# ChikaYan/mvs_gaussian_splatting

Hardware: AMD Instinct MI355X
Metric: Mpixels/s fwd + train-step ms @1080p, 6M Gaussians, 1->8 MI355X (higher is better)
Workload: dtype f32

## Files before the change

### include/gsr.h

```cpp
#ifndef GSR_H_
#define GSR_H_

#include <stddef.h>
#include <stdint.h>

#ifdef __cplusplus
extern "C" {
#endif

#define GSR_ABI_VERSION 16

enum {
  GSR_OK = 0,
  GSR_E_BADARG = -1,
  GSR_E_CAPACITY = -2,
  GSR_E_ALIGN = -3
};

typedef struct GsrParams {
  int32_t P;
  int32_t M;
  int32_t D;
  int32_t width, height;
  float tan_fovx, tan_fovy;
  float scale_modifier;
  int32_t prefiltered;
  int32_t debug;
  const float* means3D;
  const float* shs;
  const float* colors_precomp;
  const float* opacities;
  const float* scales;
  const float* rotations;
  const float* cov3D_precomp;
  const float* viewmatrix;
  const float* projmatrix;
  const float* campos;
  const float* bg;
  void* profile;
  const float* shs_rest;
  int32_t act_flags;
  int32_t binning_mode;
  uint32_t* counts_pinned;
  int32_t forward_only;
  int32_t debug_flags;
  uint8_t* visible_out;
  int32_t depth_span_lt24;
} GsrParams;

enum {
  GSR_DEBUG_NO_MINIBLOCK_CULL = 1
};

enum {
  GSR_BINNING_TWO_LEVEL = 0,
  GSR_BINNING_KEYS64 = 1,
  GSR_BINNING_TWO_LEVEL_CULLED = 2
};

enum {
  GSR_ACT_SCALE_EXP = 1,
  GSR_ACT_ROT_NORMALIZE = 2,
  GSR_ACT_OPACITY_SIGMOID = 4
};

typedef struct GsrGrads {
  float* dL_dmeans3D;
  float* dL_dmeans2D;
  float* dL_dshs;
  float* dL_dcolors;
  float* dL_dopacities;
  float* dL_dscales;
  float* dL_drotations;
  float* dL_dcov3D;
  float* dL_dshs_rest;
  float* stats_xyz_gradient_accum;
  float* stats_denom;
  float* stats_max_radii2D;
} GsrGrads;

int gsr_abi_version(void);
const char* gsr_last_error(void);
const char* gsr_build_info(void);

// ... 191 lines not shown
```

### mvs_gaussian_splatting_amd/_lib.py

```python
from __future__ import annotations

import ctypes as C
import os
import threading

_HERE = os.path.dirname(os.path.abspath(__file__))
LIB_PATH = os.environ.get("GSR_LIB_PATH") or os.path.join(_HERE, "libgsr_hip.so")

ABI_VERSION = 16


class GsrParams(C.Structure):
    _fields_ = [
        ("P", C.c_int32), ("M", C.c_int32), ("D", C.c_int32),
        ("width", C.c_int32), ("height", C.c_int32),
        ("tan_fovx", C.c_float), ("tan_fovy", C.c_float), ("scale_modifier", C.c_float),
        ("prefiltered", C.c_int32), ("debug", C.c_int32),
        ("means3D", C.c_void_p), ("shs", C.c_void_p), ("colors_precomp", C.c_void_p),
        ("opacities", C.c_void_p), ("scales", C.c_void_p), ("rotations", C.c_void_p),
        ("cov3D_precomp", C.c_void_p), ("viewmatrix", C.c_void_p), ("projmatrix", C.c_void_p),
        ("campos", C.c_void_p), ("bg", C.c_void_p), ("profile", C.c_void_p),
        ("shs_rest", C.c_void_p), ("act_flags", C.c_int32), ("binning_mode", C.c_int32),
        ("counts_pinned", C.c_void_p), ("forward_only", C.c_int32), ("debug_flags", C.c_int32),
        ("visible_out", C.c_void_p), ("depth_span_lt24", C.c_int32),
    ]


class GsrGrads(C.Structure):
    _fields_ = [
        ("dL_dmeans3D", C.c_void_p), ("dL_dmeans2D", C.c_void_p), ("dL_dshs", C.c_void_p),
        ("dL_dcolors", C.c_void_p), ("dL_dopacities", C.c_void_p), ("dL_dscales", C.c_void_p),
        ("dL_drotations", C.c_void_p), ("dL_dcov3D", C.c_void_p), ("dL_dshs_rest", C.c_void_p),
        ("stats_xyz_gradient_accum", C.c_void_p), ("stats_denom", C.c_void_p), ("stats_max_radii2D", C.c_void_p),
    ]


class GsrGrow(C.Structure):
    _fields_ = [("P", C.c_int32), ("G", C.c_int32), ("mode", C.c_int32), ("num_dirs", C.c_int32), ("n_rest", C.c_int32)] + [
        (n, C.c_void_p) for n in ("xyz", "f_dc", "f_rest", "opacity", "scaling", "rotation", "dirs_prob", "dirs",
                                  "conti_dirs", "grow_dist", "split_distance", "split_scale", "noise", "vidx", "src")]


class GsrGrowGrads(C.Structure):
    _fields_ = [("in_", C.c_void_p * 7), ("out", C.c_void_p * 7)] + [
        (n, C.c_void_p) for n in ("d_dirs_prob", "d_conti_dirs", "d_grow_dist", "d_split_distance", "d_split_scale")]


GROW_DIR, GROW_CONTINUOUS, GROW_DISTANCE, SPLIT_DISTANCE, SPLIT_SCALE = 1, 2, 4, 8, 16


class GsrDensifyFork(C.Structure):
    _fields_ = [("P", C.c_int32), ("mode", C.c_int32), ("num_dirs", C.c_int32)] + [
        (n, C.c_void_p) for n in ("xyz", "scaling", "rotation", "dirs_prob", "dirs", "conti_dirs", "grow_dist",
                                  "split_distance", "split_scale", "noise", "dir_noise")]


DENSIFY_GROW, DENSIFY_SYMMETRIC = 32, 64
ROW_COPY, ROW_CONST, ROW_SKIP = 0, 1, 2


def ROW_POLICY(orig_sel: int, extra: int, child: int) -> int:
    return orig_sel | (extra << 2) | (child << 4)
ACT_SCALE_EXP, ACT_ROT_NORMALIZE, ACT_OPACITY_SIGMOID = 1, 2, 4
BINNING_TWO_LEVEL, BINNING_KEYS64, BINNING_TWO_LEVEL_CULLED = 0, 1, 2
DSSIM_ONE_MINUS_MEAN, DSSIM_CLAMPED_HALF = 0, 1
DEBUG_NO_MINIBLOCK_CULL = 1


ADAM_MAX_TENSORS = 16


class GsrAdamTensor(C.Structure):
    _fields_ = [("param", C.c_void_p), ("grad", C.c_void_p), ("exp_avg", C.c_void_p), ("exp_avg_sq", C.c_void_p),
                ("numel", C.c_int64)] + [
        (n, C.c_float) for n in ("lerp_weight", "beta2", "sq_weight", "bc2_sqrt", "eps", "step_size")]


class GsrAdamBatch(C.Structure):
    _fields_ = [("count", C.c_int32), ("reserved", C.c_int32), ("t", GsrAdamTensor * ADAM_MAX_TENSORS)]


SYMBOLS = {
    "gsr_abi_version": (C.c_int, []),
    "gsr_last_error": (C.c_char_p, []),
    "gsr_build_info": (C.c_char_p, []),
    "gsr_geom_bytes": (C.c_size_t, [C.c_int32]),
    "gsr_image_bytes": (C.c_size_t, [C.c_int32, C.c_int32]),
    "gsr_binning_bytes": (C.c_size_t, [C.c_uint32, C.c_uint32, C.c_int32, C.c_int32, C.c_int32]),
    "gsr_backward_bytes": (C.c_size_t, [C.c_int32, C.c_uint32]),
    "gsr_forward_preprocess": (C.c_int, [C.POINTER(GsrParams), C.c_void_p, C.c_void_p, C.c_void_p,
                                         C.POINTER(C.c_uint32), C.POINTER(C.c_uint32)]),
    "gsr_forward_render": (C.c_int, [C.POINTER(GsrParams), C.c_void_p, C.c_void_p, C.c_size_t, C.c_void_p,
                                     C.c_uint32, C.c_uint32, C.c_void_p, C.c_void_p]),
    "gsr_forward": (C.c_int, [C.POINTER(GsrParams), C.c_void_p, C.c_void_p, C.c_size_t, C.c_uint32, C.c_void_p,
                              C.c_void_p, C.c_void_p, C.c_void_p, C.c_void_p]),
    "gsr_event_create": (C.c_int, [C.POINTER(C.c_void_p)]),
    "gsr_event_destroy": (C.c_int, [C.c_void_p]),
    "gsr_event_wait": (C.c_int, [C.c_void_p]),
    "gsr_event_query": (C.c_int, [C.c_void_p, C.POINTER(C.c_int32)]),
# ... 144 lines not shown
```

### mvs_gaussian_splatting_amd/csrc/gsr_api.hip

```cpp
#include <hip/hip_runtime.h>
#include <dlfcn.h>
#include <stdio.h>
#include <string.h>
#include <atomic>
#include <mutex>
#include <string>
#include <vector>

#include "gsr_common.h"
#include "gsr_launch.h"

using namespace gsr;

namespace {
thread_local std::string g_err = "";

int fail(int code, const char* msg) {
  g_err = msg;
  return code;
}
int hip_fail(hipError_t e, const char* where) {
  g_err = std::string(where) + ": " + hipGetErrorString(e);
  return (int)e;
}
// ... 441 lines not shown
                 uint32_t R, uint32_t V, const float* dL_dout_color, void* bwd_ws, size_t bwd_ws_bytes,
                 const GsrGrads* grads, void* stream) {
  if (p && p->forward_only) return fail(GSR_E_BADARG, "the forward ran with forward_only = 1: no state for a backward");
  if (int rc = validate(p)) return rc;
  if (!grads) return fail(GSR_E_BADARG, "grads is NULL");
  if (p->P == 0) return 0;
  if (!radii || !geom_ws || !img_ws || !dL_dout_color || !bwd_ws) return fail(GSR_E_BADARG, "NULL workspace / input");
  if (!grads->dL_dmeans3D || !grads->dL_dmeans2D || !grads->dL_dopacities)
    return fail(GSR_E_BADARG, "dL_dmeans3D / dL_dmeans2D / dL_dopacities must be non-NULL");
  if (p->shs && !grads->dL_dshs) return fail(GSR_E_BADARG, "dL_dshs required with shs");
  if (p->shs_rest && !grads->dL_dshs_rest) return fail(GSR_E_BADARG, "dL_dshs_rest required with shs_rest");
  if (p->shs_rest && ((uintptr_t)grads->dL_dshs_rest & 15u) != 0) return fail(GSR_E_ALIGN, "dL_dshs_rest must be 16-byte aligned");
  if (p->shs && !p->shs_rest && p->M == 16 && ((uintptr_t)grads->dL_dshs & 15u) != 0)
    return fail(GSR_E_ALIGN, "dL_dshs must be 16-byte aligned");
  if (p->colors_precomp && !grads->dL_dcolors) return fail(GSR_E_BADARG, "dL_dcolors required with colors_precomp");
  {
    const int n_stats = (grads->stats_xyz_gradient_accum != nullptr) + (grads->stats_denom != nullptr) +
                        (grads->stats_max_radii2D != nullptr);
    if (n_stats != 0 && n_stats != 3) return fail(GSR_E_BADARG, "the three stats_* pointers must be given together");
  }
  const BwdLayout Wl(p->P, R);
  if (bwd_ws_bytes < Wl.bytes) return fail(GSR_E_CAPACITY, "backward workspace too small");
  if (((uintptr_t)bwd_ws & 255u) != 0) return fail(GSR_E_ALIGN, "bwd_ws must be 256-byte aligned");
  hipStream_t s = static_cast<hipStream_t>(stream);
  const GeomLayout L(p->P);
  const ImageLayout I(p->width, p->height);
  GradRow* rows = at<GradRow>(bwd_ws, Wl.rows);
  uint8_t* flags = at<uint8_t>(bwd_ws, Wl.flags);
  const GeomRec* rec = at<GeomRec>(geom_ws, L.rec);
  if (R > 0) {
    if (!bin_ws) return fail(GSR_E_BADARG, "bin_ws is NULL");
    const SortedViews sv = sorted_views(bin_ws, R, V, p->width, p->height, p->binning_mode);
    const uint32_t* point_list = sv.point_list;
    GSR_HIP(hipMemsetAsync(flags, 0, R, s));
    {
      StageTimer t(p, GSR_STAGE_RENDER_BWD, s);
      launch_render_bwd(p->width, p->height, at<uint2>(img_ws, I.ranges), point_list, rec,
                        at<uint32_t>(geom_ws, L.slot_base), p->bg,
                        at<float>(img_ws, I.final_T), at<uint32_t>(img_ws, I.n_contrib),
                        at<uint32_t>(img_ws, I.tile_max), dL_dout_color, rows, flags,
                        at<uint32_t>(img_ws, I.tile_order), s, sv.inst_mask);
    }
    if (int rc = check(p, s, "render_bwd")) return rc;
  }
  {
    StageTimer t(p, GSR_STAGE_PREPROCESS_BWD, s);
    launch_sum_big_rows(at<uint32_t>(geom_ws, L.total) + TOTAL_BIG, at<uint32_t>(geom_ws, L.block_big_offs), L.nblocks,
                        at<uint32_t>(geom_ws, L.big_list), rec, at<uint32_t>(geom_ws, L.slot_base), rows, flags, s);
    launch_preprocess_bwd(*p, radii, rec, at<uint32_t>(geom_ws, L.slot_base), rows, flags, *grads, s);
  }
  return check(p, s, "preprocess_bwd");
}

int gsr_profile_create(void** handle) {
  if (!handle) return fail(GSR_E_BADARG, "handle is NULL");
  *handle = new Profile();
  return 0;
}
int gsr_profile_destroy(void* handle) {
  Profile* pr = static_cast<Profile*>(handle);
  if (!pr) return 0;
  for (auto& sp : pr->used) { if (sp.a) (void)hipEventDestroy(sp.a); if (sp.b) (void)hipEventDestroy(sp.b); }
  for (auto e : pr->pool) (void)hipEventDestroy(e);
  delete pr;
  return 0;
}
int gsr_profile_collect(void* handle, double* ms_sum, uint32_t* counts) {
  Profile* pr = static_cast<Profile*>(handle);
  if (!pr || !ms_sum || !counts) return fail(GSR_E_BADARG, "NULL argument");
  std::vector<Profile::Span> spans;
  {
    std::lock_guard<std::mutex> lock(pr->mu);
    spans.swap(pr->used);
  }
// ... 400 lines not shown
```

### mvs_gaussian_splatting_amd/csrc/gsr_common.h

```cpp
#pragma once
#include <hip/hip_runtime.h>
#include <stdint.h>
#include "../../include/gsr.h"

namespace gsr {

constexpr int TILE = 16;
constexpr int WAVE = 64;
constexpr float NEAR_Z = 0.2f;
constexpr float DILATION = 0.3f;
constexpr float FOV_GUARD = 1.3f;
constexpr float ALPHA_MAX = 0.99f;
constexpr float ALPHA_MIN = 1.0f / 255.0f;
constexpr float T_STOP = 0.0001f;

struct __attribute__((aligned(64))) GeomRec {
  float x, y, cxx, cxy;
  float cyy, opacity, r, g;
  float b, ext_x, ext_y;
  uint32_t tile_mask;
  uint32_t rect_min;
  uint32_t rect_wh;
  float kk;
  float isyy;
// ... 145 lines not shown
};

struct BinLayout {
  size_t keys_a, keys_b, vals_a, vals_b;
  size_t bsum2, boffs2, itile_a, itile_b, ig_a, ig_b;
  size_t sort, bytes;
  uint32_t nblocks2;
  __host__ __device__ BinLayout(uint32_t R, uint32_t V, int mode) {
    const size_t n = R ? R : 1, v = V ? V : 1;
    nblocks2 = (uint32_t)((v + PRE_BLOCK - 1) / PRE_BLOCK);
    size_t o = 0;
    keys_a = keys_b = vals_a = vals_b = 0;
    bsum2 = boffs2 = itile_a = itile_b = ig_a = ig_b = 0;
    if (mode == 1) {
      keys_a = o; o = align_up(o + 8 * n, 256);
      keys_b = o; o = align_up(o + 8 * n, 256);
      vals_a = o; o = align_up(o + 4 * n, 256);
      vals_b = o; o = align_up(o + 4 * n, 256);
      sort = o;   o = align_up(o + SortLayout((uint32_t)n).bytes, 256);
    } else {
      bsum2 = o;  o = align_up(o + 4 * (size_t)(nblocks2 + 1), 256);
      boffs2 = o; o = align_up(o + 4 * (size_t)(nblocks2 + 1) + 64, 256);
      itile_a = o; o = align_up(o + 4 * n, 256);
      itile_b = o; o = align_up(o + 4 * n, 256);
      ig_a = o;   o = align_up(o + 4 * n, 256);
      ig_b = o;   o = align_up(o + 4 * n, 256);
      sort = o;   o = align_up(o + SortLayout((uint32_t)n).bytes, 256);
    }
    bytes = o;
  }
};

struct BwdLayout {
  size_t rows, flags, bytes;
  __host__ __device__ BwdLayout(int P, uint32_t R) {
    (void)P;
    size_t n = R ? R : 1;
    size_t o = 0;
    rows = o;  o = align_up(o + sizeof(GradRow) * n, 256);
    flags = o; o = align_up(o + n, 256);
    bytes = o;
  }
};

__host__ __device__ inline int tile_bits(int tiles) {
  int b = 0;
  while ((1 << b) < tiles) ++b;
  return b;
}

__host__ __device__ inline int tile_sort_bits(int tiles) { const int b = tile_bits(tiles); return b < 1 ? 1 : b; }

__device__ inline float qmin_rect(float cxx, float cxy, float cyy, float icxx, float icyy, float dx0, float dx1,
                                  float dy0, float dy1) {
#pragma clang fp contract(fast)
  const float xe = fminf(dx1, fmaxf(dx0, 0.0f)), ye = fminf(dy1, fmaxf(dy0, 0.0f));
  const float yv = fminf(dy1, fmaxf(dy0, -cxy * xe * icyy));
  const float xh = fminf(dx1, fmaxf(dx0, -cxy * ye * icxx));
  const float qv = cxx * xe * xe + (2.0f * cxy * xe + cyy * yv) * yv;
  const float qh = cyy * ye * ye + (2.0f * cxy * ye + cxx * xh) * xh;
  return (xe == 0.0f && ye == 0.0f) ? 0.0f : fminf(xe != 0.0f ? qv : qh, ye != 0.0f ? qh : qv);
}

__device__ inline float densify_grad_norm(float gx, float gy) { return sqrtf(__builtin_fmaf(gx, gx, gy * gy)); }

__device__ inline int lane_id() { return __builtin_amdgcn_mbcnt_hi(~0u, __builtin_amdgcn_mbcnt_lo(~0u, 0)); }

__device__ inline uint32_t wave_incl_scan_u32(uint32_t v) {
  const int lane = lane_id();
#pragma unroll
  for (int d = 1; d < WAVE; d <<= 1) {
    uint32_t o = __shfl_up(v, d, WAVE);
    if (lane >= d) v += o;
// ... 18 lines not shown
```

### mvs_gaussian_splatting_amd/csrc/gsr_launch.h

```cpp
#pragma once
#include "gsr_common.h"

namespace gsr {

void launch_preprocess_fwd(const GsrParams& p, GeomRec* rec, BinInfo* bin, uint32_t* block_sums, uint32_t* block_vis,
                           int32_t* radii, uint32_t* block_big, uint32_t* big_list, uint2* block_range, hipStream_t s);
void launch_sum_big_rows(const uint32_t* big_count, const uint32_t* big_offs, int nb, const uint32_t* big_list,
                         const GeomRec* rec, const uint32_t* slot_base, GradRow* rows, uint8_t* row_flags, hipStream_t s);
void launch_scan_block_sums(const uint32_t* sums_a, uint32_t* offs_a, uint32_t* total_a, const uint32_t* sums_b,
                            uint32_t* offs_b, uint32_t* total_b, int nb, hipStream_t s,
                            uint32_t* host_mirror = nullptr, const uint2* block_range = nullptr,
                            const uint32_t* sums_c = nullptr, uint32_t* offs_c = nullptr, uint32_t* total_c = nullptr);
void launch_preprocess_bwd(const GsrParams& p, const int32_t* radii, const GeomRec* rec, const uint32_t* slot_base,
                           const GradRow* rows,
                           const uint8_t* row_flags, const GsrGrads& g, hipStream_t s);

void launch_duplicate_with_keys(int P, int grid_x, const BinInfo* bin, const uint32_t* block_offs, uint32_t* slot_base,
                                uint32_t* point_offsets, uint64_t* keys, uint32_t* vals, hipStream_t s);
bool launch_sort_pairs(uint64_t* keys_a, uint32_t* vals_a, uint64_t* keys_b, uint32_t* vals_b, uint32_t n,
                       int end_bit, void* scratch, hipStream_t s);
struct SortedRuns {
  uint2* runs_rel;
  uint32_t n_keys;
  bool valid;
// ... 4 lines not shown
bool launch_sort_pairs_u32(uint32_t* keys_a, uint32_t* vals_a, uint32_t* keys_b, uint32_t* vals_b, uint32_t n,
                           int end_bit, void* scratch, hipStream_t s, const uint32_t* n_dev = nullptr,
                           SortedRuns* runs = nullptr);
void launch_identify_tile_ranges_u32(uint32_t R, const uint32_t* tiles, uint2* ranges, hipStream_t s,
                                     const uint32_t* r_dev = nullptr);
inline int sort_passes(int end_bit) { return (end_bit + RADIX_BITS - 1) / RADIX_BITS; }
void launch_identify_tile_ranges(uint32_t R, const uint64_t* keys, uint2* ranges, hipStream_t s);
void launch_build_tile_order(int tiles, const uint2* ranges, uint32_t* order, hipStream_t s);
void launch_ranges_and_order_from_sort(int tiles, const SortedRuns& sr, uint2* ranges, uint32_t* order, hipStream_t s);
void launch_compact_visible(int P, const BinInfo* bin, const uint32_t* block_vis_offs, const uint32_t* block_offs,
                            uint32_t* slot_base, uint32_t* total, uint32_t capacity, int grid_x, uint32_t* dkey,
                            uint2* dval, hipStream_t s, bool top_pass_enqueued = true);
bool launch_sort_pairs_u32_v64(uint32_t* keys_a, uint2* vals_a, uint32_t* keys_b, uint2* vals_b, uint32_t n,
                               int end_bit, void* scratch, hipStream_t s, const uint32_t* n_dev = nullptr);
void launch_sort_extra_pass_u32(const uint32_t* kin, const uint2* vin, uint32_t* kout, uint2* vout, uint32_t n,
                                const uint32_t* n_dev, int shift, int nbits, void* scratch, hipStream_t s);
void launch_count_tiles(uint32_t v_cap, const uint32_t* total, const uint2* d3, const uint2* d4, const BinInfo* bin,
                        uint32_t* block_sums2, hipStream_t s);
constexpr uint32_t EMIT_WIDE_MAX_BLOCKS = 512;
inline bool emit_is_wide(uint32_t v_cap) { return (v_cap + PRE_BLOCK - 1) / PRE_BLOCK <= EMIT_WIDE_MAX_BLOCKS; }
void launch_emit_instances(uint32_t v_cap, const uint32_t* total, int grid_x, const uint2* d3, const uint2* d4,
                           const BinInfo* bin, const uint32_t* block_offs2, uint32_t* inst_tile, uint32_t* inst_g,
                           uint32_t capacity, hipStream_t s);
void launch_reconstruct_keys(uint32_t R, uint32_t P, const uint32_t* tile_sorted, const uint32_t* point_list,
                             const BinInfo* bin, uint64_t* keys, hipStream_t s);

void launch_render_fwd(int W, int H, const uint2* ranges, const uint32_t* point_list, const GeomRec* rec,
                       const float* bg, float* out_color, float* final_T, uint32_t* n_contrib, uint32_t* tile_max,
                       const uint32_t* tile_order, hipStream_t s, unsigned long long* stats, int cull, uint16_t* inst_mask);
void launch_render_bwd(int W, int H, const uint2* ranges, const uint32_t* point_list, const GeomRec* rec,
                       const uint32_t* slot_base,
                       const float* bg, const float* final_T, const uint32_t* n_contrib, const uint32_t* tile_max,
                       const float* dL_dpix, GradRow* rows, uint8_t* row_flags, const uint32_t* tile_order,
                       hipStream_t s, const uint16_t* inst_mask);

void launch_l1_dssim(const float* x, const float* gt, int C, int H, int W, float lambda, int dssim_mode, float* sums,
                     float* dL_dx, float* maps, hipStream_t s);

struct Splat2dLayout {
  size_t rec, flag, pre, gmask, partial, bytes;
  int chunks, per_chunk;
  Splat2dLayout(int N, int H, int W);
};
int splat2d_max_kernel_size();
void launch_splat2d_fwd(int N, int K, int H, int W, const float* sx, const float* sy, const float* rho,
                        const float* coords, const float* colours, const float* ax, void* ws, float* out,
                        hipStream_t s);
void launch_splat2d_bwd(int N, int K, int H, int W, const float* sx, const float* sy, const float* rho, const float* ax,
                        void* ws, const float* dL_dout, float* d_sx, float* d_sy, float* d_rho, float* d_coords,
                        float* d_colours, hipStream_t s);

struct GrowLayout {
  size_t flags, block_counts, block_offs, totals, bytes;
  int nblocks;
  explicit GrowLayout(int P);
};
void launch_grow_plan(int P, const float* accum, const float* denom, const float* scaling, float thr, float pde,
                      int split_mode, void* ws, int32_t* vidx, int32_t* src, uint8_t* selected, hipStream_t s);
void launch_grow_expand(const GsrGrow& g, float* const out[6], hipStream_t s);
void launch_grow_fold(const GsrGrow& g, const GsrGrowGrads& d, hipStream_t s);

struct DensifyLayout {
  size_t flags, block_counts, block_offs, totals, pos, bytes;
  int nblocks;
  explicit DensifyLayout(int P);
};
void launch_densify_plan(int P, const float* accum, const float* denom, const float* scaling, const float* opacity,
// ... 37 lines not shown
```

### mvs_gaussian_splatting_amd/csrc/render.hip

```cpp
#include "gsr_common.h"
#include "gsr_launch.h"
#include <type_traits>

namespace gsr {

constexpr int BATCH = WAVE;
constexpr int WAVES_PER_BLOCK = 4;
constexpr float LOG2E = 1.4426950408889634f;

struct Staged {
  float4 q0, q1, q2;
  float kk, isyy;
  uint32_t rect_min, rect_wh, slot_base;
};

__device__ inline void load_staged(const GeomRec* __restrict__ rec, uint32_t id, Staged& s) {
  const float* f0 = reinterpret_cast<const float*>(rec + id);
  const float* f = f0 + 4;
  s.q0.x = f0[0];
  s.q0.y = f0[1];
  s.q0.z = f0[2];
  s.q1.y = f[1];
  s.q1.z = f[2];
  s.q1.w = f[3];
  s.q2.x = f[4];
  s.q2.y = f[5];
  s.q2.z = f[6];
  const float2 k = *reinterpret_cast<const float2*>(reinterpret_cast<const char*>(rec + id) + 56);
  s.kk = k.x;
  s.isyy = k.y;
}

struct LdsRec {
  float4 A;
// ... 237 lines not shown
  if (TRACK) {
    uint32_t mx = inside ? last : 0u;
#pragma unroll
    for (int d = WAVE / 2; d > 0; d >>= 1) mx = max(mx, (uint32_t)__shfl_xor((int)mx, d, WAVE));
    if (lane == 0) sFlag[1][wid] = mx;
    __syncthreads();
    if (tid == 0) tile_max[tile] = max(max(sFlag[1][0], sFlag[1][1]), max(sFlag[1][2], sFlag[1][3]));
  }
  if (STATS) {
    st_pairs = (unsigned long long)wave_reduce_add_u32((uint32_t)st_pairs);
    if (lane == 0) {
      atomicAdd(&stats[2], st_pairs);
      atomicAdd(&stats[3], st_evals);
    }
    if (tid == 0) {
      atomicAdd(&stats[0], (unsigned long long)len);
      atomicAdd(&stats[1], (unsigned long long)min(len, ((len + QROUND - 1) / QROUND) * QROUND));
      if (TRACK) atomicAdd(&stats[5], (unsigned long long)max(max(sFlag[1][0], sFlag[1][1]), max(sFlag[1][2], sFlag[1][3])));
    }
  }
}

constexpr int MB_DUMMY = WAVE;
#ifdef BWD_PROFILE
__device__ unsigned long long g_bwd_prof[8];
#define PROF_T(x) const unsigned long long x = __builtin_readcyclecounter()
#define PROF_ADD(k, a, b) prof[k] += (unsigned long long)((b) - (a))
#define PROF_CNT(k, n) prof[k] += (unsigned long long)(n)
#else
#define PROF_T(x)
#define PROF_ADD(k, a, b)
#define PROF_CNT(k, n)
#endif
constexpr int MB_WIN = 26;
constexpr int MB_LIST = MB_WIN + 4;
constexpr int DYN_CAP = 253;
struct MbLds {
  struct Rec { float4 A, B; float C; float pad[3]; } R[WAVE + 1];
  __attribute__((aligned(16))) uint16_t list[16][MB_LIST];
  float4 s0[DYN_CAP + 2];
  float4 s1[DYN_CAP + 2];
  float s2[DYN_CAP + 2];
#ifdef BWD_LDS_PAD
  char occupancy_probe[BWD_LDS_PAD];
#endif
};
static_assert((16 * MB_LIST * 2) % 16 == 0 && 16 * MB_LIST * 2 / 16 <= WAVE, "the list block is padded by one 16-byte store per lane");

__device__ __forceinline__ void quad_fold9(float (&v)[9]) {
  asm volatile(
      "s_nop 1\n\t"
      "v_add_f32_dpp %0, %0, %0 quad_perm:[1,0,3,2] row_mask:0xf bank_mask:0xf\n\t"
      "v_add_f32_dpp %1, %1, %1 quad_perm:[1,0,3,2] row_mask:0xf bank_mask:0xf\n\t"
      "v_add_f32_dpp %2, %2, %2 quad_perm:[1,0,3,2] row_mask:0xf bank_mask:0xf\n\t"
      "v_add_f32_dpp %3, %3, %3 quad_perm:[1,0,3,2] row_mask:0xf bank_mask:0xf\n\t"
      "v_add_f32_dpp %4, %4, %4 quad_perm:[1,0,3,2] row_mask:0xf bank_mask:0xf\n\t"
      "v_add_f32_dpp %5, %5, %5 quad_perm:[1,0,3,2] row_mask:0xf bank_mask:0xf\n\t"
      "v_add_f32_dpp %6, %6, %6 quad_perm:[1,0,3,2] row_mask:0xf bank_mask:0xf\n\t"
      "v_add_f32_dpp %7, %7, %7 quad_perm:[1,0,3,2] row_mask:0xf bank_mask:0xf\n\t"
      "v_add_f32_dpp %8, %8, %8 quad_perm:[1,0,3,2] row_mask:0xf bank_mask:0xf\n\t"
      "v_add_f32_dpp %0, %0, %0 quad_perm:[2,3,0,1] row_mask:0xf bank_mask:0xf\n\t"
      "v_add_f32_dpp %1, %1, %1 quad_perm:[2,3,0,1] row_mask:0xf bank_mask:0xf\n\t"
      "v_add_f32_dpp %2, %2, %2 quad_perm:[2,3,0,1] row_mask:0xf bank_mask:0xf\n\t"
      "v_add_f32_dpp %3, %3, %3 quad_perm:[2,3,0,1] row_mask:0xf bank_mask:0xf\n\t"
      "v_add_f32_dpp %4, %4, %4 quad_perm:[2,3,0,1] row_mask:0xf bank_mask:0xf\n\t"
      "v_add_f32_dpp %5, %5, %5 quad_perm:[2,3,0,1] row_mask:0xf bank_mask:0xf\n\t"
      "v_add_f32_dpp %6, %6, %6 quad_perm:[2,3,0,1] row_mask:0xf bank_mask:0xf\n\t"
      "v_add_f32_dpp %7, %7, %7 quad_perm:[2,3,0,1] row_mask:0xf bank_mask:0xf\n\t"
      "v_add_f32_dpp %8, %8, %8 quad_perm:[2,3,0,1] row_mask:0xf bank_mask:0xf"
      : "+v"(v[0]), "+v"(v[1]), "+v"(v[2]), "+v"(v[3]), "+v"(v[4]), "+v"(v[5]), "+v"(v[6]), "+v"(v[7]), "+v"(v[8]));
}

__device__ __forceinline__ void render_bwd_tile_mb16(const int tile, MbLds& L, int W, int H, int grid_x,
                                                     const uint2* __restrict__ ranges,
                                                     const uint32_t* __restrict__ point_list,
                                                     const GeomRec* __restrict__ rec,
                                                     const uint16_t* __restrict__ inst_mask,
                                                     const uint32_t* __restrict__ slot_base, const float* __restrict__ bg,
// ... 59 lines not shown
    st.q1.y = f[5]; st.q1.z = f[6]; st.q1.w = f[7]; st.q2.x = f[8];
    st.q2.w = f[11];
    const uint4 rr = *reinterpret_cast<const uint4*>(base + 48);
    st.rect_min = rr.x;
    st.rect_wh = rr.y;
    st.kk = __uint_as_float(rr.z);
    st.isyy = __uint_as_float(rr.w);
    st.slot_base = slot_base[id];
  };
  auto load_mask = [&](uint32_t lo, uint32_t top) { return (uint32_t)inst_mask[start + min(lo + lane, top - 1)]; };
  uint32_t mask_next = 0;
  uint32_t lo = hi > BATCH ? hi - BATCH : 0u;
  uint32_t id_next = 0;
  if (hi > 0) {
    load_rec(load_id(lo, hi));
    mask_next = load_mask(lo, hi);
    const uint32_t lo2 = lo > BATCH ? lo - BATCH : 0u;
    id_next = load_id(lo2, max(lo, 1u));
  }

  bool pending = false;
  uint32_t p_slot = 0u, p_base = 0u, p_cnt = 0u;
  uint32_t p_chunks = 1u;
  float p_lo2op = 0.0f;
  auto flush_rows = [&]() {
    __builtin_amdgcn_wave_barrier();
    {
      float r9[9] = {0.f, 0.f, 0.f, 0.f, 0.f, 0.f, 0.f, 0.f, 0.f};
      auto chunk = [&](const uint32_t c0) {
        float4 f[4], g[4];
        float hh[4];
#pragma unroll
        for (int t = 0; t < 4; ++t) {
#ifdef BWD_EXP_FLUSH_SLOT0
          const uint32_t at = (c0 + t < p_cnt) ? 0u : 0u;
#else
          const uint32_t at = (c0 + t < p_cnt) ? p_base + c0 + t : 0u;
#endif
          f[t] = L.s0[at];
          g[t] = L.s1[at];
          hh[t] = L.s2[at];
        }
#pragma unroll
        for (int t = 0; t < 4; ++t) {
          r9[0] += f[t].x; r9[1] += f[t].y; r9[2] += f[t].z; r9[3] += f[t].w;
          r9[4] += g[t].x; r9[5] += g[t].y; r9[6] += g[t].z; r9[7] += g[t].w;
          r9[8] += hh[t];
        }
      };
      chunk(0u);
      if (p_chunks > 1u) chunk(4u);
      if (p_chunks > 2u) chunk(8u);
      if (p_chunks > 3u) chunk(12u);
      uint32_t bits = 0u;
#pragma unroll
      for (int t = 0; t < 9; ++t) bits |= __float_as_uint(r9[t]);
      const bool nz = (bits << 1) != 0u;
#ifdef BWD_EXP_NO_ROWWRITE
      if (nz && (bits & 0x3ffu) == 0x155u) {
#else
      if (nz) {
#endif
        GradRow t;
        t.dmx = r9[0]; t.dmy = r9[1]; t.dcxx = -0.5f * r9[2]; t.dcxy = -r9[3];
        t.dcyy = -0.5f * r9[4]; t.dop = r9[5] * __builtin_amdgcn_exp2f(-p_lo2op); t.dr = r9[6]; t.dg = r9[7];
        t.db = r9[8];
        rows[p_slot] = t;
        row_flags[p_slot] = 1;
      }
    }
    __builtin_amdgcn_wave_barrier();
  };
#ifdef BWD_PROFILE
  unsigned long long prof[8] = {0, 0, 0, 0, 0, 0, 0, 0};
#endif
  PROF_T(t_tile0);
  while (hi > 0) {
    PROF_T(t_r0);
    PROF_CNT(4, 1);
    const uint32_t cur_lo = lo;
    const bool have = lo + lane < hi;
    const uint32_t active = (uint32_t)__builtin_amdgcn_ballot_w64(mbl > cur_lo);
    const uint32_t m = have ? (mask_next & active) : 0u;
    const bool clamp = __builtin_amdgcn_ballot_w64(m != 0u && st.q1.y > ALPHA_MAX) != 0ull;
    const uint32_t rw = st.rect_wh & 0xffffu;
    const uint32_t bit = ((uint32_t)tile_y - rect_min_y(st.rect_min)) * rw + ((uint32_t)tile_x - rect_min_x(st.rect_min));
    const uint32_t slot = st.slot_base + bin_rank(st.rect_wh, __float_as_uint(st.q2.w), have ? bit : 0u);
    LdsRec lr;
    make_lds(st, lr);
    const float lo2op = lr.B.y;
    __builtin_amdgcn_wave_barrier();
    L.R[lane].A = lr.A;
    L.R[lane].B = lr.B;
    L.R[lane].C = st.q2.x;
    hi = lo;
// ... 24 lines not shown
      const uint32_t cnt = (uint32_t)__popc(mr);
      const uint32_t cincl = wave_incl_scan_dpp(cnt);
      const uint32_t above = (uint32_t)__builtin_amdgcn_readlane((int)cincl, WAVE - 1) - cincl;
      const bool inA = rem && (over & 0x80808080u) == 0u && above + cnt <= (uint32_t)DYN_CAP;
      const unsigned long long balA = __builtin_amdgcn_ballot_w64(inA);
      uint32_t nmax;
      {
        const int cA = __builtin_ctzll(balA);
        const uint32_t c0 = (uint32_t)__builtin_amdgcn_readlane((int)sfx[0], cA), c1 = (uint32_t)__builtin_amdgcn_readlane((int)sfx[1], cA);
        const uint32_t c2 = (uint32_t)__builtin_amdgcn_readlane((int)sfx[2], cA), c3 = (uint32_t)__builtin_amdgcn_readlane((int)sfx[3], cA);
        const uint32_t csel = (lane & 8) ? ((lane & 4) ? c3 : c2) : ((lane & 4) ? c1 : c0);
        uint32_t len = (csel >> (8 * (lane & 3))) & 0xffu;
        len = max(len, (uint32_t)__builtin_amdgcn_update_dpp(0, (int)len, 0x128, 0xf, 0xf, false));
        len = max(len, (uint32_t)__builtin_amdgcn_update_dpp(0, (int)len, 0x124, 0xf, 0xf, false));
        len = max(len, (uint32_t)__builtin_amdgcn_update_dpp(0, (int)len, 0x122, 0xf, 0xf, false));
        len = max(len, (uint32_t)__builtin_amdgcn_update_dpp(0, (int)len, 0x121, 0xf, 0xf, false));
        nmax = (uint32_t)__builtin_amdgcn_readlane((int)len, 0);
      }
      uint32_t idx[4];
#pragma unroll
      for (int r = 0; r < 4; ++r) idx[r] = inA ? (sfx[r] & (own[r] * 0xffu)) : 0u;
      __builtin_amdgcn_wave_barrier();
      {
        const uint32_t dd = ((uint32_t)MB_DUMMY | ((uint32_t)(DYN_CAP + 1) << 8)) * 0x10001u;
        uint4* l4 = reinterpret_cast<uint4*>(&L.list[0][0]);
        if (lane < 16 * MB_LIST * 2 / 16) l4[lane] = make_uint4(dd, dd, dd, dd);
      }
      __builtin_amdgcn_wave_barrier();
#pragma unroll
      for (int r = 0; r < 4; ++r)
#pragma unroll
        for (int k = 0; k < 4; ++k) {
          const uint32_t sl = above + 1u + (uint32_t)__popc(m & ((1u << (4 * r + k)) - 1u));
#ifdef BWD_EXP_LIST_PRED
          const uint32_t pp = (idx[r] >> (8 * k)) & 0xffu;
          if (pp) L.list[4 * r + k][pp] = (uint16_t)((sl << 8) | (uint32_t)lane);
#else
          L.list[4 * r + k][(idx[r] >> (8 * k)) & 0xffu] = (uint16_t)((sl << 8) | (uint32_t)lane);
#endif
        }
      __builtin_amdgcn_wave_barrier();
      auto walk = [&](auto clamped_c) {
        constexpr bool CLAMPED = decltype(clamped_c)::value;
        auto fetch = [&](uint32_t e, float4& a, float4& b, float& cb) {
#ifdef BWD_EXP_REC_BANK
          const char* rp = reinterpret_cast<const char*>(L.R) + 48u * ((e & 0u) + (uint32_t)mb);
#else
          const char* rp = reinterpret_cast<const char*>(L.R) + 48u * (e & 0xffu);
#endif
          a = *reinterpret_cast<const float4*>(rp);
          b = *reinterpret_cast<const float4*>(rp + 16);
          cb = *reinterpret_cast<const float*>(rp + 32);
        };
        auto step = [&](const float4 a, const float4 b, const float cb, const uint32_t e0, const uint32_t i) {
          const uint32_t pos1 = cur_lo + (e0 & 0xffu) + 1u;
          float v[9] = {0.f, 0.f, 0.f, 0.f, 0.f, 0.f, 0.f, 0.f, 0.f};
          float S = 0.f, Sx = 0.f, Sy = 0.f, Sxy = 0.f;
#pragma unroll
          for (int k = 0; k < 4; ++k) {
            const float dx = a.x - ((k & 1) ? pxf1 : pxf0), dy = a.y - ((k >> 1) ? pyf1 : pyf0);
            const float ar = __builtin_amdgcn_exp2f(pair_p2(dx, dy, a.z, a.w, b.x, b.y));
            const bool ok = pos1 <= last[k] && ar >= ALPHA_MIN;
            const float arm = ok ? ar : 0.0f;
            const float am = CLAMPED ? clamp_alpha(arm, b.x) : arm;
            const float rcp = __builtin_amdgcn_rcpf(1.0f - am);
            T[k] *= rcp;
            const float D = fmaf(cb, dpb[k], fmaf(b.w, dpg[k], fmaf(b.z, dpr[k], -U[k])));
            const float dch = am * T[k];
            const float h = (CLAMPED ? arm * T[k] : dch) * D;
            U[k] = fmaf(am, D, U[k]);
            S += h;
            if (k & 1) Sx += h;
            if (k >> 1) Sy += h;
            if (k == 3) Sxy = h;
            v[6] = fmaf(dch, dpr[k], v[6]); v[7] = fmaf(dch, dpg[k], v[7]); v[8] = fmaf(dch, dpb[k], v[8]);
          }
          {
            const float dx0 = a.x - pxf0, dy0 = a.y - pyf0;
            v[0] = fmaf(dx0, S, -Sx);
            v[1] = fmaf(dy0, S, -Sy);
            v[2] = fmaf(dx0, v[0] - Sx, Sx);
            v[4] = fmaf(dy0, v[1] - Sy, Sy);
            v[3] = fmaf(dx0, v[1], fmaf(-dy0, Sx, Sxy));
            v[5] = S;
          }
          quad_fold9(v);
#ifdef BWD_EXP_SLOT_LANE
          L.s0[1 + mb] = make_float4(v[0], v[1], v[2], v[3]);
          L.s1[1 + mb] = make_float4(v[4], v[5], v[6], v[7]);
          L.s2[1 + mb] = v[8];
#else
          L.s0[e0 >> 8] = make_float4(v[0], v[1], v[2], v[3]);
          L.s1[e0 >> 8] = make_float4(v[4], v[5], v[6], v[7]);
          L.s2[e0 >> 8] = v[8];
#endif
        };
        uint32_t e0 = mylist[0], e1 = mylist[1];
        float4 a, b, an, bn;
        float cb, cbn;
        fetch(e0, a, b, cb);
        for (uint32_t i = 0; i < nmax; ++i) {
          fetch(e1, an, bn, cbn);
          const uint32_t e2 = mylist[i + 2];
          step(a, b, cb, e0, i);
          e0 = e1; e1 = e2;
          a = an; b = bn; cb = cbn;
        }
      };
      PROF_T(t_p1);
      PROF_ADD(1, t_p0, t_p1);
      PROF_CNT(6, nmax);
#ifndef BWD_EXP_NO_FLUSH
      if (pending) flush_rows();
#endif
      PROF_T(t_p1b);
      PROF_ADD(3, t_p1, t_p1b);
      if (clamp) walk(std::true_type{}); else walk(std::false_type{});
      __builtin_amdgcn_wave_barrier();
      PROF_T(t_p2);
      PROF_ADD(2, t_p1b, t_p2);
      pending = true;
      p_slot = slot;
      p_lo2op = lo2op;
      p_base = above + 1u;
      p_cnt = inA ? cnt : 0u;
      p_chunks = 1u + (__builtin_amdgcn_ballot_w64(p_cnt > 4u) != 0ull ? 1u : 0u) + (__builtin_amdgcn_ballot_w64(p_cnt > 8u) != 0ull ? 1u : 0u) +
                 (__builtin_amdgcn_ballot_w64(p_cnt > 12u) != 0ull ? 1u : 0u);
      remaining &= ~balA;
    }
  }
  if (pending) flush_rows();
#ifdef BWD_PROFILE
  {
    PROF_T(t_tile1);
    prof[7] = t_tile1 - t_tile0;
    if (lane == 0)
      for (int k = 0; k < 8; ++k) atomicAdd(&g_bwd_prof[k], prof[k]);
  }
#endif
}

constexpr int BWD_WAVES = 3;
__global__ __launch_bounds__(WAVES_PER_BLOCK * WAVE, BWD_WAVES) void render_bwd_kernel(int W, int H, int grid_x, int num_tiles,
                                                          const uint32_t* __restrict__ tile_order,
                                                          const uint2* __restrict__ ranges,
                                                          const uint32_t* __restrict__ point_list,
                                                          const GeomRec* __restrict__ rec,
                                                          const uint16_t* __restrict__ inst_mask,
                                                          const uint32_t* __restrict__ slot_base,
                                                          const float* __restrict__ bg,
                                                          const float* __restrict__ final_T,
                                                          const uint32_t* __restrict__ n_contrib,
                                                          const uint32_t* __restrict__ tile_max,
                                                          const float* __restrict__ dL_dpix,
                                                          GradRow* __restrict__ rows,
                                                          uint8_t* __restrict__ row_flags) {
  __shared__ MbLds sL[WAVES_PER_BLOCK];
  const int wid = __builtin_amdgcn_readfirstlane((int)(threadIdx.x / WAVE));
  const int slot = blockIdx.x * WAVES_PER_BLOCK + wid;
  if (slot >= num_tiles) return;
  const int tile = __builtin_amdgcn_readfirstlane((int)tile_order[slot]);
  render_bwd_tile_mb16(tile, sL[wid], W, H, grid_x, ranges, point_list, rec, inst_mask, slot_base, bg, final_T, n_contrib, tile_max,
                       dL_dpix, rows, row_flags);
}

void launch_render_fwd(int W, int H, const uint2* ranges, const uint32_t* point_list, const GeomRec* rec,
                       const float* bg, float* out_color, float* final_T, uint32_t* n_contrib, uint32_t* tile_max,
                       const uint32_t* tile_order, hipStream_t s, unsigned long long* stats, int cull, uint16_t* inst_mask) {
  const int gx = (W + TILE - 1) / TILE, gy = (H + TILE - 1) / TILE;
  const int nblk = gx * gy;
  if (stats)
    hipLaunchKernelGGL((render_fwd_kernel<true, true>), dim3(nblk), dim3(256), 0, s, W, H, gx, cull, tile_order, ranges,
                       point_list, rec, bg, out_color, final_T, n_contrib, tile_max, inst_mask, stats);
  else if (final_T && n_contrib && tile_max)
    hipLaunchKernelGGL((render_fwd_kernel<false, true>), dim3(nblk), dim3(256), 0, s, W, H, gx, cull, tile_order, ranges,
                       point_list, rec, bg, out_color, final_T, n_contrib, tile_max, inst_mask, stats);
  else
    hipLaunchKernelGGL((render_fwd_kernel<false, false>), dim3(nblk), dim3(256), 0, s, W, H, gx, cull, tile_order, ranges,
                       point_list, rec, bg, out_color, final_T, n_contrib, tile_max, inst_mask, stats);
}
#ifdef BWD_PROFILE
extern "C" int gsr_debug_bwd_profile(unsigned long long* out8, int reset) {
  if (hipDeviceSynchronize() != hipSuccess) return 1;
  if (hipMemcpyFromSymbol(out8, HIP_SYMBOL(g_bwd_prof), 64) != hipSuccess) return 2;
  if (reset) {
    unsigned long long z[8] = {0, 0, 0, 0, 0, 0, 0, 0};
    if (hipMemcpyToSymbol(HIP_SYMBOL(g_bwd_prof), z, 64) != hipSuccess) return 3;
  }
  return 0;
}
#endif
void launch_render_bwd(int W, int H, const uint2* ranges, const uint32_t* point_list, const GeomRec* rec,
                       const uint32_t* slot_base, const float* bg, const float* final_T, const uint32_t* n_contrib, const uint32_t* tile_max,
                       const float* dL_dpix, GradRow* rows, uint8_t* row_flags, const uint32_t* tile_order,
                       hipStream_t s, const uint16_t* inst_mask) {
  const int gx = (W + TILE - 1) / TILE, gy = (H + TILE - 1) / TILE;
  const int nblk = (gx * gy + WAVES_PER_BLOCK - 1) / WAVES_PER_BLOCK;
  hipLaunchKernelGGL(render_bwd_kernel, dim3(nblk), dim3(WAVES_PER_BLOCK * WAVE), 0, s, W, H, gx, gx * gy, tile_order, ranges, point_list, rec,
                     inst_mask, slot_base, bg, final_T, n_contrib, tile_max, dL_dpix, rows, row_flags);
}

}
```

Before: 2333.

## Use persistent ticket-based dynamic tile scheduling in backward render kernel

The backward render kernel now launches only as many blocks as can be resident (CUs times the occupancy bound). Each wave grabs further tiles from a global atomic ticket counter instead of owning one fixed tile, which replaces the fixed one-tile-per-wave mapping. Wave priority is set high for the first tiles and lowered for later ones. The aim is to cut tail imbalance when per-tile cost varies widely, at the price of an atomic per tile, an extra memset covering the ticket, and a static fallback kept under a debug flag. Dead experimental ifdefs are removed and optional timeline instrumentation is added.

```diff
diff --git a/include/gsr.h b/include/gsr.h
--- a/include/gsr.h
+++ b/include/gsr.h
@@ -8,7 +8,7 @@
 extern "C" {
 #endif
 
-#define GSR_ABI_VERSION 16
+#define GSR_ABI_VERSION 17
 
 enum {
   GSR_OK = 0,
@@ -49,7 +49,8 @@
 } GsrParams;
 
 enum {
-  GSR_DEBUG_NO_MINIBLOCK_CULL = 1
+  GSR_DEBUG_NO_MINIBLOCK_CULL = 1,
+  GSR_DEBUG_STATIC_TILE_SCHEDULE = 2
 };
 
 enum {
diff --git a/mvs_gaussian_splatting_amd/_lib.py b/mvs_gaussian_splatting_amd/_lib.py
--- a/mvs_gaussian_splatting_amd/_lib.py
+++ b/mvs_gaussian_splatting_amd/_lib.py
@@ -7,7 +7,7 @@
 _HERE = os.path.dirname(os.path.abspath(__file__))
 LIB_PATH = os.environ.get("GSR_LIB_PATH") or os.path.join(_HERE, "libgsr_hip.so")
 
-ABI_VERSION = 16
+ABI_VERSION = 17
 
 
 class GsrParams(C.Structure):
@@ -65,6 +65,7 @@
 BINNING_TWO_LEVEL, BINNING_KEYS64, BINNING_TWO_LEVEL_CULLED = 0, 1, 2
 DSSIM_ONE_MINUS_MEAN, DSSIM_CLAMPED_HALF = 0, 1
 DEBUG_NO_MINIBLOCK_CULL = 1
+DEBUG_STATIC_TILE_SCHEDULE = 2
 
 
 ADAM_MAX_TENSORS = 16
diff --git a/mvs_gaussian_splatting_amd/csrc/gsr_api.hip b/mvs_gaussian_splatting_amd/csrc/gsr_api.hip
--- a/mvs_gaussian_splatting_amd/csrc/gsr_api.hip
+++ b/mvs_gaussian_splatting_amd/csrc/gsr_api.hip
@@ -497,14 +497,15 @@
     if (!bin_ws) return fail(GSR_E_BADARG, "bin_ws is NULL");
     const SortedViews sv = sorted_views(bin_ws, R, V, p->width, p->height, p->binning_mode);
     const uint32_t* point_list = sv.point_list;
-    GSR_HIP(hipMemsetAsync(flags, 0, R, s));
+    GSR_HIP(hipMemsetAsync(flags, 0, Wl.ticket + 4 - Wl.flags, s));
     {
       StageTimer t(p, GSR_STAGE_RENDER_BWD, s);
       launch_render_bwd(p->width, p->height, at<uint2>(img_ws, I.ranges), point_list, rec,
                         at<uint32_t>(geom_ws, L.slot_base), p->bg,
                         at<float>(img_ws, I.final_T), at<uint32_t>(img_ws, I.n_contrib),
                         at<uint32_t>(img_ws, I.tile_max), dL_dout_color, rows, flags,
-                        at<uint32_t>(img_ws, I.tile_order), s, sv.inst_mask);
+                        at<uint32_t>(img_ws, I.tile_order), s, sv.inst_mask,
+                        (p->debug_flags & GSR_DEBUG_STATIC_TILE_SCHEDULE) ? nullptr : at<uint32_t>(bwd_ws, Wl.ticket));
     }
     if (int rc = check(p, s, "render_bwd")) return rc;
   }
diff --git a/mvs_gaussian_splatting_amd/csrc/gsr_common.h b/mvs_gaussian_splatting_amd/csrc/gsr_common.h
--- a/mvs_gaussian_splatting_amd/csrc/gsr_common.h
+++ b/mvs_gaussian_splatting_amd/csrc/gsr_common.h
@@ -201,13 +201,14 @@
 };
 
 struct BwdLayout {
-  size_t rows, flags, bytes;
+  size_t rows, flags, ticket, bytes;
   __host__ __device__ BwdLayout(int P, uint32_t R) {
     (void)P;
     size_t n = R ? R : 1;
     size_t o = 0;
     rows = o;  o = align_up(o + sizeof(GradRow) * n, 256);
     flags = o; o = align_up(o + n, 256);
+    ticket = o; o = align_up(o + 4, 256);
     bytes = o;
   }
 };
diff --git a/mvs_gaussian_splatting_amd/csrc/gsr_launch.h b/mvs_gaussian_splatting_amd/csrc/gsr_launch.h
--- a/mvs_gaussian_splatting_amd/csrc/gsr_launch.h
+++ b/mvs_gaussian_splatting_amd/csrc/gsr_launch.h
@@ -60,7 +60,7 @@
                        const uint32_t* slot_base,
                        const float* bg, const float* final_T, const uint32_t* n_contrib, const uint32_t* tile_max,
                        const float* dL_dpix, GradRow* rows, uint8_t* row_flags, const uint32_t* tile_order,
-                       hipStream_t s, const uint16_t* inst_mask);
+                       hipStream_t s, const uint16_t* inst_mask, uint32_t* ticket);
 
 void launch_l1_dssim(const float* x, const float* gt, int C, int H, int W, float lambda, int dssim_mode, float* sums,
                      float* dL_dx, float* maps, hipStream_t s);
diff --git a/mvs_gaussian_splatting_amd/csrc/render.hip b/mvs_gaussian_splatting_amd/csrc/render.hip
--- a/mvs_gaussian_splatting_amd/csrc/render.hip
+++ b/mvs_gaussian_splatting_amd/csrc/render.hip
@@ -1,5 +1,7 @@
 #include "gsr_common.h"
 #include "gsr_launch.h"
+#include <algorithm>
+#include <atomic>
 #include <type_traits>
 
 namespace gsr {
@@ -303,6 +305,24 @@
 #define PROF_ADD(k, a, b)
 #define PROF_CNT(k, n)
 #endif
+#if defined(BWD_PROFILE) || defined(BWD_TIMELINE)
+constexpr int BWD_TL_CAP = 16384;
+struct BwdTlRec { uint32_t tile, hw_id, xcc_id, pad; unsigned long long t0, t1; };
+__device__ BwdTlRec g_bwd_tl[BWD_TL_CAP];
+#define BWD_TL_BEGIN(slot, tile)                                                                      \
+  if ((threadIdx.x & (WAVE - 1)) == 0 && (uint32_t)(slot) < (uint32_t)BWD_TL_CAP) {                   \
+    BwdTlRec& r_ = g_bwd_tl[slot];                                                                    \
+    r_.tile = (uint32_t)(tile);                                                                       \
+    r_.hw_id = __builtin_amdgcn_s_getreg(4 | (31 << 11));              \
+    r_.xcc_id = __builtin_amdgcn_s_getreg(20 | (31 << 11));                        \
+    r_.t0 = wall_clock64();                                                                           \
+  }
+#define BWD_TL_END(slot)                                                                              \
+  if ((threadIdx.x & (WAVE - 1)) == 0 && (uint32_t)(slot) < (uint32_t)BWD_TL_CAP) g_bwd_tl[slot].t1 = wall_clock64()
+#else
+#define BWD_TL_BEGIN(slot, tile)
+#define BWD_TL_END(slot)
+#endif
 constexpr int MB_WIN = 26;
 constexpr int MB_LIST = MB_WIN + 4;
 constexpr int DYN_CAP = 253;
@@ -312,9 +332,6 @@
   float4 s0[DYN_CAP + 2];
   float4 s1[DYN_CAP + 2];
   float s2[DYN_CAP + 2];
-#ifdef BWD_LDS_PAD
-  char occupancy_probe[BWD_LDS_PAD];
-#endif
 };
 static_assert((16 * MB_LIST * 2) % 16 == 0 && 16 * MB_LIST * 2 / 16 <= WAVE, "the list block is padded by one 16-byte store per lane");
 
@@ -440,11 +457,7 @@
         float hh[4];
 #pragma unroll
         for (int t = 0; t < 4; ++t) {
-#ifdef BWD_EXP_FLUSH_SLOT0
-          const uint32_t at = (c0 + t < p_cnt) ? 0u : 0u;
-#else
           const uint32_t at = (c0 + t < p_cnt) ? p_base + c0 + t : 0u;
-#endif
           f[t] = L.s0[at];
           g[t] = L.s1[at];
           hh[t] = L.s2[at];
@@ -464,11 +477,7 @@
 #pragma unroll
       for (int t = 0; t < 9; ++t) bits |= __float_as_uint(r9[t]);
       const bool nz = (bits << 1) != 0u;
-#ifdef BWD_EXP_NO_ROWWRITE
-      if (nz && (bits & 0x3ffu) == 0x155u) {
-#else
       if (nz) {
-#endif
         GradRow t;
         t.dmx = r9[0]; t.dmy = r9[1]; t.dcxx = -0.5f * r9[2]; t.dcxy = -r9[3];
         t.dcyy = -0.5f * r9[4]; t.dop = r9[5] * __builtin_amdgcn_exp2f(-p_lo2op); t.dr = r9[6]; t.dg = r9[7];
@@ -559,22 +568,13 @@
 #pragma unroll
         for (int k = 0; k < 4; ++k) {
           const uint32_t sl = above + 1u + (uint32_t)__popc(m & ((1u << (4 * r + k)) - 1u));
-#ifdef BWD_EXP_LIST_PRED
-          const uint32_t pp = (idx[r] >> (8 * k)) & 0xffu;
-          if (pp) L.list[4 * r + k][pp] = (uint16_t)((sl << 8) | (uint32_t)lane);
-#else
           L.list[4 * r + k][(idx[r] >> (8 * k)) & 0xffu] = (uint16_t)((sl << 8) | (uint32_t)lane);
-#endif
         }
       __builtin_amdgcn_wave_barrier();
       auto walk = [&](auto clamped_c) {
         constexpr bool CLAMPED = decltype(clamped_c)::value;
         auto fetch = [&](uint32_t e, float4& a, float4& b, float& cb) {
-#ifdef BWD_EXP_REC_BANK
-          const char* rp = reinterpret_cast<const char*>(L.R) + 48u * ((e & 0u) + (uint32_t)mb);
-#else
           const char* rp = reinterpret_cast<const char*>(L.R) + 48u * (e & 0xffu);
-#endif
           a = *reinterpret_cast<const float4*>(rp);
           b = *reinterpret_cast<const float4*>(rp + 16);
           cb = *reinterpret_cast<const float*>(rp + 32);
@@ -612,15 +612,9 @@
             v[5] = S;
           }
           quad_fold9(v);
-#ifdef BWD_EXP_SLOT_LANE
-          L.s0[1 + mb] = make_float4(v[0], v[1], v[2], v[3]);
-          L.s1[1 + mb] = make_float4(v[4], v[5], v[6], v[7]);
-          L.s2[1 + mb] = v[8];
-#else
           L.s0[e0 >> 8] = make_float4(v[0], v[1], v[2], v[3]);
           L.s1[e0 >> 8] = make_float4(v[4], v[5], v[6], v[7]);
           L.s2[e0 >> 8] = v[8];
-#endif
         };
         uint32_t e0 = mylist[0], e1 = mylist[1];
         float4 a, b, an, bn;
@@ -637,9 +631,7 @@
       PROF_T(t_p1);
       PROF_ADD(1, t_p0, t_p1);
       PROF_CNT(6, nmax);
-#ifndef BWD_EXP_NO_FLUSH
       if (pending) flush_rows();
-#endif
       PROF_T(t_p1b);
       PROF_ADD(3, t_p1, t_p1b);
       if (clamp) walk(std::true_type{}); else walk(std::false_type{});
@@ -668,7 +660,9 @@
 }
 
 constexpr int BWD_WAVES = 3;
+template <bool TICKET>
 __global__ __launch_bounds__(WAVES_PER_BLOCK * WAVE, BWD_WAVES) void render_bwd_kernel(int W, int H, int grid_x, int num_tiles,
+                                                          uint32_t* __restrict__ ticket,
                                                           const uint32_t* __restrict__ tile_order,
                                                           const uint2* __restrict__ ranges,
                                                           const uint32_t* __restrict__ point_list,
@@ -684,11 +678,32 @@
                                                           uint8_t* __restrict__ row_flags) {
   __shared__ MbLds sL[WAVES_PER_BLOCK];
   const int wid = __builtin_amdgcn_readfirstlane((int)(threadIdx.x / WAVE));
-  const int slot = blockIdx.x * WAVES_PER_BLOCK + wid;
-  if (slot >= num_tiles) return;
-  const int tile = __builtin_amdgcn_readfirstlane((int)tile_order[slot]);
-  render_bwd_tile_mb16(tile, sL[wid], W, H, grid_x, ranges, point_list, rec, inst_mask, slot_base, bg, final_T, n_contrib, tile_max,
-                       dL_dpix, rows, row_flags);
+  if (TICKET) {
+    const uint32_t grid_waves = gridDim.x * WAVES_PER_BLOCK;
+    uint32_t slot = blockIdx.x * WAVES_PER_BLOCK + wid;
+    for (int taken = 0; slot < (uint32_t)num_tiles; ++taken) {
+      if (taken == 0) __builtin_amdgcn_s_setprio(3);
+      else if (taken == 1) __builtin_amdgcn_s_setprio(2);
+      else if (taken == 2) __builtin_amdgcn_s_setprio(1);
+      else __builtin_amdgcn_s_setprio(0);
+      const int tile = __builtin_amdgcn_readfirstlane((int)tile_order[slot]);
+      BWD_TL_BEGIN(slot, tile);
+      render_bwd_tile_mb16(tile, sL[wid], W, H, grid_x, ranges, point_list, rec, inst_mask, slot_base, bg, final_T, n_contrib,
+                           tile_max, dL_dpix, rows, row_flags);
+      BWD_TL_END(slot);
+      uint32_t t = 0u;
+      if ((threadIdx.x & (WAVE - 1)) == 0) t = atomicAdd(ticket, 1u);
+      slot = grid_waves + (uint32_t)__builtin_amdgcn_readfirstlane((int)t);
+    }
+  } else {
+    const int slot = blockIdx.x * WAVES_PER_BLOCK + wid;
+    if (slot >= num_tiles) return;
+    const int tile = __builtin_amdgcn_readfirstlane((int)tile_order[slot]);
+    BWD_TL_BEGIN(slot, tile);
+    render_bwd_tile_mb16(tile, sL[wid], W, H, grid_x, ranges, point_list, rec, inst_mask, slot_base, bg, final_T, n_contrib, tile_max,
+                         dL_dpix, rows, row_flags);
+    BWD_TL_END(slot);
+  }
 }
 
 void launch_render_fwd(int W, int H, const uint2* ranges, const uint32_t* point_list, const GeomRec* rec,
@@ -717,14 +732,41 @@
   return 0;
 }
 #endif
+#if defined(BWD_PROFILE) || defined(BWD_TIMELINE)
+extern "C" int gsr_debug_bwd_timeline_cap(void) { return BWD_TL_CAP; }
+extern "C" int gsr_debug_bwd_timeline(void* out, int n) {
+  if (n < 0 || n > BWD_TL_CAP) return 4;
+  if (hipDeviceSynchronize() != hipSuccess) return 1;
+  if (hipMemcpyFromSymbol(out, HIP_SYMBOL(g_bwd_tl), sizeof(BwdTlRec) * (size_t)n) != hipSuccess) return 2;
+  return 0;
+}
+#endif
+static int bwd_resident_blocks() {
+  constexpr int MAX_DEV = 64;
+  static std::atomic<int> cus[MAX_DEV];
+  int d = 0;
+  if (hipGetDevice(&d) != hipSuccess || d < 0 || d >= MAX_DEV) d = -1;
+  int n = d >= 0 ? cus[d].load(std::memory_order_relaxed) : 0;
+  if (n == 0) {
+    hipDeviceProp_t prop;
+    n = (d >= 0 && hipGetDeviceProperties(&prop, d) == hipSuccess && prop.multiProcessorCount > 0) ? prop.multiProcessorCount : 256;
+    if (d >= 0) cus[d].store(n, std::memory_order_relaxed);
+  }
+  return BWD_WAVES * n;
+}
 void launch_render_bwd(int W, int H, const uint2* ranges, const uint32_t* point_list, const GeomRec* rec,
                        const uint32_t* slot_base, const float* bg, const float* final_T, const uint32_t* n_contrib, const uint32_t* tile_max,
                        const float* dL_dpix, GradRow* rows, uint8_t* row_flags, const uint32_t* tile_order,
-                       hipStream_t s, const uint16_t* inst_mask) {
+                       hipStream_t s, const uint16_t* inst_mask, uint32_t* ticket) {
   const int gx = (W + TILE - 1) / TILE, gy = (H + TILE - 1) / TILE;
   const int nblk = (gx * gy + WAVES_PER_BLOCK - 1) / WAVES_PER_BLOCK;
-  hipLaunchKernelGGL(render_bwd_kernel, dim3(nblk), dim3(WAVES_PER_BLOCK * WAVE), 0, s, W, H, gx, gx * gy, tile_order, ranges, point_list, rec,
-                     inst_mask, slot_base, bg, final_T, n_contrib, tile_max, dL_dpix, rows, row_flags);
-}
-
-}
+  if (ticket)
+    hipLaunchKernelGGL(render_bwd_kernel<true>, dim3(std::min(nblk, bwd_resident_blocks())), dim3(WAVES_PER_BLOCK * WAVE), 0, s, W, H, gx,
+                       gx * gy, ticket, tile_order, ranges, point_list, rec, inst_mask, slot_base, bg, final_T, n_contrib, tile_max,
+                       dL_dpix, rows, row_flags);
+  else
+    hipLaunchKernelGGL(render_bwd_kernel<false>, dim3(nblk), dim3(WAVES_PER_BLOCK * WAVE), 0, s, W, H, gx, gx * gy, ticket, tile_order,
+                       ranges, point_list, rec, inst_mask, slot_base, bg, final_T, n_contrib, tile_max, dL_dpix, rows, row_flags);
+}
+
+}
```

New measurement: 2333, median of 5. No clear change (+0.0%).
